# BrByte/brb_framework

Measured on AMD Instinct MI355X. Metric: GiB/s (device-resident) + Mrecords/s over 1500B buffers at 1/2/4/8 MI355X, higher is better.
Workload: dtype u32

## Files before the change

### brb_framework_amd/csrc/gpu/digest_line.h

```cpp
#pragma once

#include "dma_stage.h"
#include "test_options.h"

#ifndef BRB_LINE_PROBE
#define BRB_LINE_PROBE_DECL
#define BRB_LINE_PROBE(ev) ((void)0)
#endif

namespace brb_digest {

template <class Alg, bool OUT_ALIGNED, bool TAIL_HI>
BRB_DEV void line_finish(typename Alg::State &st, const uint32_t (&w0)[16], const uint32_t (&w1)[16],
                         const uint32_t (&tm)[16], const uint32_t (&tp)[16], uint32_t t, uint32_t rec_len,
                         uint8_t *out, uint64_t r, uint64_t n_rec)
{
    if (t == 0) {
        Alg::pad_only(st, rec_len);
        if (r < n_rec)
            Alg::template store<OUT_ALIGNED>(out, r, st);
        return;
    }
    uint32_t w[16];
#pragma unroll
    for (int i = 0; i < 16; i++)
        w[i] = ((TAIL_HI ? w1[i] : w0[i]) & tm[i]) | tp[i];
    Alg::finish(st, w, t, rec_len);
    if (r < n_rec)
        Alg::template store<OUT_ALIGNED>(out, r, st);
}

BRB_DEV void tail_masks(uint32_t t, uint32_t (&tm)[16], uint32_t (&tp)[16])
{
#pragma unroll
    for (uint32_t i = 0; i < 16; i++) {
        const uint32_t o = 4 * i;
        const uint32_t keep = t > o ? (t - o < 4 ? t - o : 4) : 0;
        tm[i] = uint32_t((uint64_t(1) << (8 * keep)) - 1);
        tp[i] = t >= o && t < o + 4 ? 0x80u << (8 * (t - o)) : 0u;
        asm volatile("" : "+v"(tm[i]), "+v"(tp[i]));
    }
}

inline bool line_tail_hi(uint32_t rec_len)
{
    return ((rec_len >> 6) & 1) != 0;
}

template <class Alg, int WAVES, bool OUT_ALIGNED, bool TAIL_HI>
__global__ __launch_bounds__(64 * WAVES, 2) void digest_line_kernel(const uint8_t *__restrict__ data,
                                                                             uint32_t rec_len, uint64_t n_rec,
                                                                             uint8_t *__restrict__ out)
{
    constexpr uint32_t SLOT = 8192;
    __shared__ __attribute__((aligned(16))) uint8_t ring[WAVES * 2 * SLOT];
    __shared__ uint32_t next_ticket;
    const uint32_t lane = threadIdx.x & 63;
    const uint32_t wv = __builtin_amdgcn_readfirstlane(threadIdx.x >> 6);
    [[maybe_unused]] const uint64_t wave0 = uint64_t(blockIdx.x) * WAVES + wv;
    const uint64_t n_groups = (n_rec + 63) / 64;
    if (threadIdx.x == 0)
        next_ticket = WAVES;
    __syncthreads();
    auto take = [&]() -> uint64_t {
        uint32_t tk = 0;
        if (lane == 0)
            tk = __hip_atomic_fetch_add(&next_ticket, 1u, __ATOMIC_RELAXED, __HIP_MEMORY_SCOPE_WORKGROUP);
        tk = __builtin_amdgcn_readfirstlane(tk);
        return uint64_t(blockIdx.x) + uint64_t(tk) * gridDim.x;
    };
    uint64_t g = uint64_t(blockIdx.x) + uint64_t(wv) * gridDim.x;
    if (g >= n_groups)
        return;
    const uint32_t my_off = wv * 2 * SLOT;
    const uint32_t lds0 = uint32_t(reinterpret_cast<uintptr_t>(ring)) + my_off;
    const uint32_t nfull = rec_len >> 6, t = rec_len & 63;
    const uint32_t nblk = nfull + (t ? 1 : 0);
    const uint32_t K = (nblk + 1) >> 1;
    const uint32_t P = (K & 1) ^ 1;
    const uint64_t dbase = reinterpret_cast<uint64_t>(data);
    const uint64_t end_line = (dbase + n_rec * rec_len + 127) & ~uint64_t(127);
    const uint64_t gbytes = uint64_t(rec_len) * 64;
    const uint32_t o0 = uint32_t(dbase) & 127;
    auto swz = [](uint32_t row) { return (row >> 1) & 7; };

    uint32_t vq[8];
    {
        const uint32_t l3 = lane >> 3;
        const uint32_t base = o0 + l3 * rec_len;
        const uint32_t g0 = 16u * ((lane & 7) ^ (l3 >> 1));
#pragma unroll
        for (int q = 0; q < 8; q++) {
            const uint32_t x = base + 8u * q * rec_len;
            vq[q] = ((x & ~127u) | (q & 1 ? g0 ^ 64u : g0)) + (4096u - 1024u * (q & 3));
        }
    }
    brb_dma::v4i rs, rsn;
    auto desc = [&](uint64_t g, brb_dma::v4i &rs) {
        const uint64_t gbase = ((dbase + g * gbytes) & ~uint64_t(127)) - 4096;
        const uint64_t gleft = end_line - gbase;
        rs.x = __builtin_amdgcn_readfirstlane(int(uint32_t(gbase)));
        rs.y = __builtin_amdgcn_readfirstlane(int(uint32_t(gbase >> 32) & 0xFFFF));
        rs.z = __builtin_amdgcn_readfirstlane(int(gleft > 0x7FFFFFFFull ? 0x7FFFFFFFu : uint32_t(gleft)));
        rs.w = 0x00020000;
    };
    uint32_t so = 0, son = 0;
    auto issue = [&](const brb_dma::v4i &rs, uint32_t &so, uint32_t slot, bool keep_l2 = false) {
#ifdef BRB_LINE_NO_DMA
        return;
#endif
        const uint32_t m = lds0 + slot * SLOT;
        uint32_t keep;
#define BRB_LINE_DMA8(POL)                                                                      \
    asm volatile("s_mov_b32 %0, m0\n\t"                                                          \
                 "s_mov_b32 m0, %10\n\t"                                                         \
                 "s_nop 0\n\t"                                                                   \
                 "buffer_load_dwordx4 %1, %9, %12 offen " POL "lds\n\t"                         \
                 "buffer_load_dwordx4 %2, %9, %12 offen offset:1024 " POL "lds\n\t"             \
                 "buffer_load_dwordx4 %3, %9, %12 offen offset:2048 " POL "lds\n\t"             \
                 "buffer_load_dwordx4 %4, %9, %12 offen offset:3072 " POL "lds\n\t"             \
                 "s_mov_b32 m0, %11\n\t"                                                         \
                 "s_nop 0\n\t"                                                                   \
                 "buffer_load_dwordx4 %5, %9, %12 offen " POL "lds\n\t"                         \
                 "buffer_load_dwordx4 %6, %9, %12 offen offset:1024 " POL "lds\n\t"             \
                 "buffer_load_dwordx4 %7, %9, %12 offen offset:2048 " POL "lds\n\t"             \
                 "buffer_load_dwordx4 %8, %9, %12 offen offset:3072 " POL "lds\n\t"             \
                 "s_mov_b32 m0, %0"                                                               \
                 : "=&s"(keep)                                                                    \
                 : "v"(vq[0]), "v"(vq[1]), "v"(vq[2]), "v"(vq[3]), "v"(vq[4]), "v"(vq[5]), "v"(vq[6]), \
                   "v"(vq[7]), "s"(rs), "s"(m), "s"(m + 4096u), "s"(so)                           \
                 : "memory")
        if (!keep_l2)
            BRB_LINE_DMA8("nt ");
        else
            BRB_LINE_DMA8("");
#undef BRB_LINE_DMA8
        so += 128;
    };

    uint32_t ae[32], ao[32];

    uint32_t w0[16], w1[16];
    auto read_window = [&](const uint32_t (&ad)[32]) {
#pragma unroll
        for (int i = 0; i < 16; i++) {
            w0[i] = *reinterpret_cast<const uint32_t *>(ring + ad[i]);
            w1[i] = *reinterpret_cast<const uint32_t *>(ring + ad[16 + i]);
        }
        __builtin_amdgcn_s_waitcnt(0xC07F);
    };

    BRB_LINE_PROBE_DECL
    BRB_LINE_PROBE(0);
    desc(g, rs);
    issue(rs, so, P, true);
    issue(rs, so, P ^ 1, true);
    __builtin_amdgcn_sched_barrier(0);
    uint64_t gn = take();
    {
        const uint32_t sh4 = (o0 + lane * rec_len) & 127;
        const uint32_t fr = (my_off + lane * 128) | (swz(lane) << 4);
#pragma unroll
        for (uint32_t i = 0; i < 32; i++) {
            const uint32_t q4 = sh4 + 4 * i;
            ae[i] = ((q4 & 124u) ^ fr) | ((q4 & 128u) << 6);
            ao[i] = ae[i] ^ SLOT;
            asm volatile("" : "+v"(ae[i]), "+v"(ao[i]));
        }
    }
    uint32_t tm[16], tp[16];
    tail_masks(t, tm, tp);
    auto full_step = [&](typename Alg::State &st, const uint32_t (&ad)[32], uint32_t refill_slot) {
        BRB_LINE_PROBE(1);
        brb_dma::wait_vmcnt<0>();
        read_window(ad);
        BRB_LINE_PROBE(2);
        issue(rs, so, refill_slot);
        __builtin_amdgcn_sched_barrier(0);
        Alg::compress(st, w0);
        Alg::compress(st, w1);
        __builtin_amdgcn_sched_barrier(0);
    };
    for (;;) {
        typename Alg::State st = Alg::iv();
        uint32_t k = 1;
        if (P) {
            full_step(st, ao, 1);
            k = 2;
        }
        for (; k + 2 <= K; k += 2) {
            full_step(st, ae, 0);
            full_step(st, ao, 1);
        }
        {
            BRB_LINE_PROBE(1);
            brb_dma::wait_vmcnt<0>();
            read_window(ae);
            BRB_LINE_PROBE(2);
            if (gn < n_groups) {
                desc(gn, rsn);
                son = 0;
                issue(rsn, son, P, true);
                issue(rsn, son, P ^ 1, true);
            }
            if (2 * K - 2 < nfull)
                Alg::compress(st, w0);
            if (2 * K - 1 < nfull)
                Alg::compress(st, w1);
        }
        line_finish<Alg, OUT_ALIGNED, TAIL_HI>(st, w0, w1, tm, tp, t, rec_len, out, g * 64 + lane, n_rec);
        g = gn;
        if (g >= n_groups)
            break;
        gn = take();
        rs = rsn;
        so = son;
    }
    BRB_LINE_PROBE(3);
}

inline bool line_supported(const uint8_t *data, uint32_t rec_len)
{
    return rec_len > 64 && rec_len <= (1u << 20) && (rec_len & 3) == 0 && (reinterpret_cast<uintptr_t>(data) & 3) == 0;
}

inline unsigned device_cu_count()
{
    static const unsigned n = [] {
        int dev = 0, c = 0;
        if (hipGetDevice(&dev) != hipSuccess || hipDeviceGetAttribute(&c, hipDeviceAttributeMultiprocessorCount, dev) != hipSuccess || c <= 0)
            c = 256;
        return unsigned(c);
    }();
    return n;
}

template <class Alg>
hipError_t launch_fixed_line(const uint8_t *data, uint32_t rec_len, uint64_t n_rec, uint8_t *out, bool out_al,
                             hipStream_t s)
{
    constexpr int W = 8;
    const uint64_t groups = (n_rec + 63) / 64;
    const unsigned g = unsigned(groups < device_cu_count() ? groups : device_cu_count());
    const bool hi = line_tail_hi(rec_len);
    if (out_al && hi)
        digest_line_kernel<Alg, W, true, true><<<g, 64 * W, 0, s>>>(data, rec_len, n_rec, out);
    else if (out_al)
        digest_line_kernel<Alg, W, true, false><<<g, 64 * W, 0, s>>>(data, rec_len, n_rec, out);
    else if (hi)
        digest_line_kernel<Alg, W, false, true><<<g, 64 * W, 0, s>>>(data, rec_len, n_rec, out);
    else
        digest_line_kernel<Alg, W, false, false><<<g, 64 * W, 0, s>>>(data, rec_len, n_rec, out);
    return hipGetLastError();
}

}
```

### brb_framework_amd/csrc/gpu/md5_device.h

```cpp
#pragma once

#include "brb_gpu_common.h"

#define BRB_MD5_F1(x, y, z) ((z) ^ ((x) & ((y) ^ (z))))
#define BRB_MD5_F2(x, y, z) ((y) ^ ((z) & ((x) ^ (y))))
#define BRB_MD5_F3(x, y, z) __builtin_amdgcn_bitop3_b32((x), (y), (z), 0x96)
#define BRB_MD5_F4(x, y, z) ((y) ^ ((x) | ~(z)))
#define BRB_MD5_STEP(F, a, b, c, d, m, k, s) (a) = (b) + rotl<s>((a) + F((b), (c), (d)) + ((m) + (k)))

struct Md5State {
    uint32_t a, b, c, d;
};

BRB_DEV Md5State md5_iv()
{
    return Md5State{0x67452301u, 0xefcdab89u, 0x98badcfeu, 0x10325476u};
}

#define BRB_MD5_STEP3X(a, b, c, d, m, k, s)                                               \
    do {                                                                                 \
        const uint32_t x_ = (a) + (m) + (k), cd_ = (c) ^ (d);                            \
        uint32_t f_;                                                                     \
        asm("v_xad_u32 %0, %1, %2, %3" : "=v"(f_) : "v"(b), "v"(cd_), "v"(x_));          \
        (a) = (b) + rotl<s>(f_);                                                         \
    } while (0)

template <bool XAD = true>
BRB_DEV void md5_compress(Md5State &st, const uint32_t (&m)[16])
{
    uint32_t a = st.a, b = st.b, c = st.c, d = st.d;

    BRB_MD5_STEP(BRB_MD5_F1, a, b, c, d, m[0], 0xd76aa478u, 7);
    BRB_MD5_STEP(BRB_MD5_F1, d, a, b, c, m[1], 0xe8c7b756u, 12);
    BRB_MD5_STEP(BRB_MD5_F1, c, d, a, b, m[2], 0x242070dbu, 17);
    BRB_MD5_STEP(BRB_MD5_F1, b, c, d, a, m[3], 0xc1bdceeeu, 22);
    BRB_MD5_STEP(BRB_MD5_F1, a, b, c, d, m[4], 0xf57c0fafu, 7);
    BRB_MD5_STEP(BRB_MD5_F1, d, a, b, c, m[5], 0x4787c62au, 12);
    BRB_MD5_STEP(BRB_MD5_F1, c, d, a, b, m[6], 0xa8304613u, 17);
    BRB_MD5_STEP(BRB_MD5_F1, b, c, d, a, m[7], 0xfd469501u, 22);
    BRB_MD5_STEP(BRB_MD5_F1, a, b, c, d, m[8], 0x698098d8u, 7);
    BRB_MD5_STEP(BRB_MD5_F1, d, a, b, c, m[9], 0x8b44f7afu, 12);
    BRB_MD5_STEP(BRB_MD5_F1, c, d, a, b, m[10], 0xffff5bb1u, 17);
    BRB_MD5_STEP(BRB_MD5_F1, b, c, d, a, m[11], 0x895cd7beu, 22);
    BRB_MD5_STEP(BRB_MD5_F1, a, b, c, d, m[12], 0x6b901122u, 7);
    BRB_MD5_STEP(BRB_MD5_F1, d, a, b, c, m[13], 0xfd987193u, 12);
    BRB_MD5_STEP(BRB_MD5_F1, c, d, a, b, m[14], 0xa679438eu, 17);
    BRB_MD5_STEP(BRB_MD5_F1, b, c, d, a, m[15], 0x49b40821u, 22);

    BRB_MD5_STEP(BRB_MD5_F2, a, b, c, d, m[1], 0xf61e2562u, 5);
    BRB_MD5_STEP(BRB_MD5_F2, d, a, b, c, m[6], 0xc040b340u, 9);
    BRB_MD5_STEP(BRB_MD5_F2, c, d, a, b, m[11], 0x265e5a51u, 14);
    BRB_MD5_STEP(BRB_MD5_F2, b, c, d, a, m[0], 0xe9b6c7aau, 20);
    BRB_MD5_STEP(BRB_MD5_F2, a, b, c, d, m[5], 0xd62f105du, 5);
    BRB_MD5_STEP(BRB_MD5_F2, d, a, b, c, m[10], 0x02441453u, 9);
    BRB_MD5_STEP(BRB_MD5_F2, c, d, a, b, m[15], 0xd8a1e681u, 14);
    BRB_MD5_STEP(BRB_MD5_F2, b, c, d, a, m[4], 0xe7d3fbc8u, 20);
    BRB_MD5_STEP(BRB_MD5_F2, a, b, c, d, m[9], 0x21e1cde6u, 5);
    BRB_MD5_STEP(BRB_MD5_F2, d, a, b, c, m[14], 0xc33707d6u, 9);
    BRB_MD5_STEP(BRB_MD5_F2, c, d, a, b, m[3], 0xf4d50d87u, 14);
    BRB_MD5_STEP(BRB_MD5_F2, b, c, d, a, m[8], 0x455a14edu, 20);
    BRB_MD5_STEP(BRB_MD5_F2, a, b, c, d, m[13], 0xa9e3e905u, 5);
    BRB_MD5_STEP(BRB_MD5_F2, d, a, b, c, m[2], 0xfcefa3f8u, 9);
    BRB_MD5_STEP(BRB_MD5_F2, c, d, a, b, m[7], 0x676f02d9u, 14);
    BRB_MD5_STEP(BRB_MD5_F2, b, c, d, a, m[12], 0x8d2a4c8au, 20);

    if constexpr (XAD) BRB_MD5_STEP3X(a, b, c, d, m[5], 0xfffa3942u, 4); else BRB_MD5_STEP(BRB_MD5_F3, a, b, c, d, m[5], 0xfffa3942u, 4);
    if constexpr (XAD) BRB_MD5_STEP3X(d, a, b, c, m[8], 0x8771f681u, 11); else BRB_MD5_STEP(BRB_MD5_F3, d, a, b, c, m[8], 0x8771f681u, 11);
    if constexpr (XAD) BRB_MD5_STEP3X(c, d, a, b, m[11], 0x6d9d6122u, 16); else BRB_MD5_STEP(BRB_MD5_F3, c, d, a, b, m[11], 0x6d9d6122u, 16);
    if constexpr (XAD) BRB_MD5_STEP3X(b, c, d, a, m[14], 0xfde5380cu, 23); else BRB_MD5_STEP(BRB_MD5_F3, b, c, d, a, m[14], 0xfde5380cu, 23);
    if constexpr (XAD) BRB_MD5_STEP3X(a, b, c, d, m[1], 0xa4beea44u, 4); else BRB_MD5_STEP(BRB_MD5_F3, a, b, c, d, m[1], 0xa4beea44u, 4);
    if constexpr (XAD) BRB_MD5_STEP3X(d, a, b, c, m[4], 0x4bdecfa9u, 11); else BRB_MD5_STEP(BRB_MD5_F3, d, a, b, c, m[4], 0x4bdecfa9u, 11);
    if constexpr (XAD) BRB_MD5_STEP3X(c, d, a, b, m[7], 0xf6bb4b60u, 16); else BRB_MD5_STEP(BRB_MD5_F3, c, d, a, b, m[7], 0xf6bb4b60u, 16);
    if constexpr (XAD) BRB_MD5_STEP3X(b, c, d, a, m[10], 0xbebfbc70u, 23); else BRB_MD5_STEP(BRB_MD5_F3, b, c, d, a, m[10], 0xbebfbc70u, 23);
    if constexpr (XAD) BRB_MD5_STEP3X(a, b, c, d, m[13], 0x289b7ec6u, 4); else BRB_MD5_STEP(BRB_MD5_F3, a, b, c, d, m[13], 0x289b7ec6u, 4);
    if constexpr (XAD) BRB_MD5_STEP3X(d, a, b, c, m[0], 0xeaa127fau, 11); else BRB_MD5_STEP(BRB_MD5_F3, d, a, b, c, m[0], 0xeaa127fau, 11);
    if constexpr (XAD) BRB_MD5_STEP3X(c, d, a, b, m[3], 0xd4ef3085u, 16); else BRB_MD5_STEP(BRB_MD5_F3, c, d, a, b, m[3], 0xd4ef3085u, 16);
    if constexpr (XAD) BRB_MD5_STEP3X(b, c, d, a, m[6], 0x04881d05u, 23); else BRB_MD5_STEP(BRB_MD5_F3, b, c, d, a, m[6], 0x04881d05u, 23);
    if constexpr (XAD) BRB_MD5_STEP3X(a, b, c, d, m[9], 0xd9d4d039u, 4); else BRB_MD5_STEP(BRB_MD5_F3, a, b, c, d, m[9], 0xd9d4d039u, 4);
    if constexpr (XAD) BRB_MD5_STEP3X(d, a, b, c, m[12], 0xe6db99e5u, 11); else BRB_MD5_STEP(BRB_MD5_F3, d, a, b, c, m[12], 0xe6db99e5u, 11);
    if constexpr (XAD) BRB_MD5_STEP3X(c, d, a, b, m[15], 0x1fa27cf8u, 16); else BRB_MD5_STEP(BRB_MD5_F3, c, d, a, b, m[15], 0x1fa27cf8u, 16);
    if constexpr (XAD) BRB_MD5_STEP3X(b, c, d, a, m[2], 0xc4ac5665u, 23); else BRB_MD5_STEP(BRB_MD5_F3, b, c, d, a, m[2], 0xc4ac5665u, 23);

    BRB_MD5_STEP(BRB_MD5_F4, a, b, c, d, m[0], 0xf4292244u, 6);
    BRB_MD5_STEP(BRB_MD5_F4, d, a, b, c, m[7], 0x432aff97u, 10);
    BRB_MD5_STEP(BRB_MD5_F4, c, d, a, b, m[14], 0xab9423a7u, 15);
    BRB_MD5_STEP(BRB_MD5_F4, b, c, d, a, m[5], 0xfc93a039u, 21);
    BRB_MD5_STEP(BRB_MD5_F4, a, b, c, d, m[12], 0x655b59c3u, 6);
    BRB_MD5_STEP(BRB_MD5_F4, d, a, b, c, m[3], 0x8f0ccc92u, 10);
    BRB_MD5_STEP(BRB_MD5_F4, c, d, a, b, m[10], 0xffeff47du, 15);
    BRB_MD5_STEP(BRB_MD5_F4, b, c, d, a, m[1], 0x85845dd1u, 21);
    BRB_MD5_STEP(BRB_MD5_F4, a, b, c, d, m[8], 0x6fa87e4fu, 6);
    BRB_MD5_STEP(BRB_MD5_F4, d, a, b, c, m[15], 0xfe2ce6e0u, 10);
    BRB_MD5_STEP(BRB_MD5_F4, c, d, a, b, m[6], 0xa3014314u, 15);
    BRB_MD5_STEP(BRB_MD5_F4, b, c, d, a, m[13], 0x4e0811a1u, 21);
    BRB_MD5_STEP(BRB_MD5_F4, a, b, c, d, m[4], 0xf7537e82u, 6);
    BRB_MD5_STEP(BRB_MD5_F4, d, a, b, c, m[11], 0xbd3af235u, 10);
    BRB_MD5_STEP(BRB_MD5_F4, c, d, a, b, m[2], 0x2ad7d2bbu, 15);
    BRB_MD5_STEP(BRB_MD5_F4, b, c, d, a, m[9], 0xeb86d391u, 21);

    st.a += a;
    st.b += b;
    st.c += c;
    st.d += d;
}

BRB_DEV void md5_finish(Md5State &st, uint32_t (&w)[16], uint32_t t, uint64_t total_len)
{
    if (t >= 56) {
        md5_compress(st, w);
#pragma unroll
        for (int i = 0; i < 14; i++)
            w[i] = 0;
    }
    w[14] = uint32_t(total_len << 3);
    w[15] = uint32_t(total_len >> 29);
    md5_compress(st, w);
}

BRB_DEV void md5_pad_only(Md5State &st, uint64_t total_len)
{
    uint32_t w[16] = {0x80u};
    w[14] = uint32_t(total_len << 3);
    w[15] = uint32_t(total_len >> 29);
    md5_compress<false>(st, w);
}
```

Baseline: 4571.

## Group records into alignment classes for vector LDS window reads; pair MD5 round-3 steps

Records are split into p alignment classes, chosen from rec_len mod 16, and each block is assigned one class. Within a class, every lane's record starts at the same 16-byte phase, so the LDS window can be read with 8-9 uint4 loads instead of 32 scalar dword loads. The phase is dispatched through compile-time specialisations, and the DMA source and window addresses are recomputed to keep the swizzle. MD5 round 3 also pairs consecutive steps so they share the b^c term. The change adds code size, more register use from the 36-word buffer, and a more complex grid mapping that could unbalance work across CUs.

```diff
diff --git a/brb_framework_amd/csrc/gpu/digest_line.h b/brb_framework_amd/csrc/gpu/digest_line.h
--- a/brb_framework_amd/csrc/gpu/digest_line.h
+++ b/brb_framework_amd/csrc/gpu/digest_line.h
@@ -1,6 +1,9 @@
 #pragma once
 
+#include <type_traits>
+
 #include "dma_stage.h"
+#include "line_layout.h"
 #include "test_options.h"
 
 #ifndef BRB_LINE_PROBE
@@ -52,13 +55,16 @@
                                                                              uint32_t rec_len, uint64_t n_rec,
                                                                              uint8_t *__restrict__ out)
 {
-    constexpr uint32_t SLOT = 8192;
+    constexpr uint32_t SLOT = brb_line_layout::kSlot;
     __shared__ __attribute__((aligned(16))) uint8_t ring[WAVES * 2 * SLOT];
     __shared__ uint32_t next_ticket;
     const uint32_t lane = threadIdx.x & 63;
     const uint32_t wv = __builtin_amdgcn_readfirstlane(threadIdx.x >> 6);
     [[maybe_unused]] const uint64_t wave0 = uint64_t(blockIdx.x) * WAVES + wv;
-    const uint64_t n_groups = (n_rec + 63) / 64;
+    const uint32_t p = brb_line_layout::period(rec_len);
+    const brb_line_layout::BlockMap bm = brb_line_layout::block_map(blockIdx.x, gridDim.x, p);
+    const uint64_t n_teams = brb_line_layout::team_count(n_rec, p);
+    const uint64_t tbytes = uint64_t(rec_len) * 64 * p;
     if (threadIdx.x == 0)
         next_ticket = WAVES;
     __syncthreads();
@@ -67,10 +73,11 @@
         if (lane == 0)
             tk = __hip_atomic_fetch_add(&next_ticket, 1u, __ATOMIC_RELAXED, __HIP_MEMORY_SCOPE_WORKGROUP);
         tk = __builtin_amdgcn_readfirstlane(tk);
-        return uint64_t(blockIdx.x) + uint64_t(tk) * gridDim.x;
-    };
-    uint64_t g = uint64_t(blockIdx.x) + uint64_t(wv) * gridDim.x;
-    if (g >= n_groups)
+        return uint64_t(bm.u) + uint64_t(tk) * bm.streams;
+    };
+    auto has_group = [&](uint64_t team) { return team < n_teams && team * 64 * p + bm.c < n_rec; };
+    uint64_t g = uint64_t(bm.u) + uint64_t(wv) * bm.streams;
+    if (!has_group(g))
         return;
     const uint32_t my_off = wv * 2 * SLOT;
     const uint32_t lds0 = uint32_t(reinterpret_cast<uintptr_t>(ring)) + my_off;
@@ -80,24 +87,18 @@
     const uint32_t P = (K & 1) ^ 1;
     const uint64_t dbase = reinterpret_cast<uint64_t>(data);
     const uint64_t end_line = (dbase + n_rec * rec_len + 127) & ~uint64_t(127);
-    const uint64_t gbytes = uint64_t(rec_len) * 64;
-    const uint32_t o0 = uint32_t(dbase) & 127;
-    auto swz = [](uint32_t row) { return (row >> 1) & 7; };
+    const uint64_t cbase = dbase + uint64_t(bm.c) * rec_len;
+    const uint32_t oc = brb_line_layout::class_off(uint32_t(dbase) & 127, bm.c, rec_len);
+    const uint32_t rstride = p * rec_len;
+    const uint32_t d = __builtin_amdgcn_readfirstlane(brb_line_layout::phase(oc));
 
     uint32_t vq[8];
-    {
-        const uint32_t l3 = lane >> 3;
-        const uint32_t base = o0 + l3 * rec_len;
-        const uint32_t g0 = 16u * ((lane & 7) ^ (l3 >> 1));
-#pragma unroll
-        for (int q = 0; q < 8; q++) {
-            const uint32_t x = base + 8u * q * rec_len;
-            vq[q] = ((x & ~127u) | (q & 1 ? g0 ^ 64u : g0)) + (4096u - 1024u * (q & 3));
-        }
-    }
+#pragma unroll
+    for (int q = 0; q < 8; q++)
+        vq[q] = brb_line_layout::dma_src(oc, rstride, q, lane) + (4096u - 1024u * (q & 3));
     brb_dma::v4i rs, rsn;
-    auto desc = [&](uint64_t g, brb_dma::v4i &rs) {
-        const uint64_t gbase = ((dbase + g * gbytes) & ~uint64_t(127)) - 4096;
+    auto desc = [&](uint64_t team, brb_dma::v4i &rs) {
+        const uint64_t gbase = ((cbase + team * tbytes) & ~uint64_t(127)) - 4096;
         const uint64_t gleft = end_line - gbase;
         rs.x = __builtin_amdgcn_readfirstlane(int(uint32_t(gbase)));
         rs.y = __builtin_amdgcn_readfirstlane(int(uint32_t(gbase >> 32) & 0xFFFF));
@@ -138,16 +139,29 @@
         so += 128;
     };
 
-    uint32_t ae[32], ao[32];
+    uint32_t ae[8], ao[8];
 
     uint32_t w0[16], w1[16];
-    auto read_window = [&](const uint32_t (&ad)[32]) {
-#pragma unroll
-        for (int i = 0; i < 16; i++) {
-            w0[i] = *reinterpret_cast<const uint32_t *>(ring + ad[i]);
-            w1[i] = *reinterpret_cast<const uint32_t *>(ring + ad[16 + i]);
+    auto read_window = [&](auto dtag, const uint32_t (&ad)[8], uint32_t ad8) {
+        constexpr int D = decltype(dtag)::value;
+        uint32_t buf[36];
+#pragma unroll
+        for (int j = 0; j < (D ? 9 : 8); j++) {
+            const uint4 v = *reinterpret_cast<const uint4 *>(ring + (j < 8 ? ad[j & 7] : ad8));
+            buf[4 * j] = v.x;
+            buf[4 * j + 1] = v.y;
+            buf[4 * j + 2] = v.z;
+            buf[4 * j + 3] = v.w;
         }
         __builtin_amdgcn_s_waitcnt(0xC07F);
+        if (D)
+            asm volatile("" : "+v"(buf[0]), "+v"(buf[1]), "+v"(buf[2]), "+v"(buf[3]), "+v"(buf[32]), "+v"(buf[33]),
+                         "+v"(buf[34]), "+v"(buf[35]));
+#pragma unroll
+        for (int i = 0; i < 16; i++) {
+            w0[i] = buf[D + i];
+            w1[i] = buf[D + 16 + i];
+        }
     };
 
     BRB_LINE_PROBE_DECL
@@ -157,64 +171,68 @@
     issue(rs, so, P ^ 1, true);
     __builtin_amdgcn_sched_barrier(0);
     uint64_t gn = take();
-    {
-        const uint32_t sh4 = (o0 + lane * rec_len) & 127;
-        const uint32_t fr = (my_off + lane * 128) | (swz(lane) << 4);
-#pragma unroll
-        for (uint32_t i = 0; i < 32; i++) {
-            const uint32_t q4 = sh4 + 4 * i;
-            ae[i] = ((q4 & 124u) ^ fr) | ((q4 & 128u) << 6);
-            ao[i] = ae[i] ^ SLOT;
-            asm volatile("" : "+v"(ae[i]), "+v"(ao[i]));
-        }
+#pragma unroll
+    for (uint32_t j = 0; j < 8; j++) {
+        ae[j] = my_off + brb_line_layout::win_addr(oc, rstride, lane, j);
+        ao[j] = ae[j] ^ SLOT;
+        asm volatile("" : "+v"(ae[j]), "+v"(ao[j]));
     }
     uint32_t tm[16], tp[16];
     tail_masks(t, tm, tp);
-    auto full_step = [&](typename Alg::State &st, const uint32_t (&ad)[32], uint32_t refill_slot) {
-        BRB_LINE_PROBE(1);
-        brb_dma::wait_vmcnt<0>();
-        read_window(ad);
-        BRB_LINE_PROBE(2);
-        issue(rs, so, refill_slot);
-        __builtin_amdgcn_sched_barrier(0);
-        Alg::compress(st, w0);
-        Alg::compress(st, w1);
-        __builtin_amdgcn_sched_barrier(0);
-    };
-    for (;;) {
-        typename Alg::State st = Alg::iv();
-        uint32_t k = 1;
-        if (P) {
-            full_step(st, ao, 1);
-            k = 2;
-        }
-        for (; k + 2 <= K; k += 2) {
-            full_step(st, ae, 0);
-            full_step(st, ao, 1);
-        }
-        {
+    auto run = [&](auto dtag) {
+        auto full_step = [&](typename Alg::State &st, const uint32_t (&ad)[8], uint32_t ad8, uint32_t refill_slot) {
             BRB_LINE_PROBE(1);
             brb_dma::wait_vmcnt<0>();
-            read_window(ae);
+            read_window(dtag, ad, ad8);
             BRB_LINE_PROBE(2);
-            if (gn < n_groups) {
-                desc(gn, rsn);
-                son = 0;
-                issue(rsn, son, P, true);
-                issue(rsn, son, P ^ 1, true);
+            issue(rs, so, refill_slot);
+            __builtin_amdgcn_sched_barrier(0);
+            Alg::compress(st, w0);
+            Alg::compress(st, w1);
+            __builtin_amdgcn_sched_barrier(0);
+        };
+        for (;;) {
+            typename Alg::State st = Alg::iv();
+            uint32_t k = 1;
+            if (P) {
+                full_step(st, ao, ae[0], 1);
+                k = 2;
             }
-            if (2 * K - 2 < nfull)
-                Alg::compress(st, w0);
-            if (2 * K - 1 < nfull)
-                Alg::compress(st, w1);
+            for (; k + 2 <= K; k += 2) {
+                full_step(st, ae, ao[0], 0);
+                full_step(st, ao, ae[0], 1);
+            }
+            {
+                BRB_LINE_PROBE(1);
+                brb_dma::wait_vmcnt<0>();
+                read_window(dtag, ae, ao[0]);
+                BRB_LINE_PROBE(2);
+                if (has_group(gn)) {
+                    desc(gn, rsn);
+                    son = 0;
+                    issue(rsn, son, P, true);
+                    issue(rsn, son, P ^ 1, true);
+                }
+                if (2 * K - 2 < nfull)
+                    Alg::compress(st, w0);
+                if (2 * K - 1 < nfull)
+                    Alg::compress(st, w1);
+            }
+            line_finish<Alg, OUT_ALIGNED, TAIL_HI>(st, w0, w1, tm, tp, t, rec_len, out,
+                                                   brb_line_layout::record_of(p, g, bm.c, lane), n_rec);
+            g = gn;
+            if (!has_group(g))
+                break;
+            gn = take();
+            rs = rsn;
+            so = son;
         }
-        line_finish<Alg, OUT_ALIGNED, TAIL_HI>(st, w0, w1, tm, tp, t, rec_len, out, g * 64 + lane, n_rec);
-        g = gn;
-        if (g >= n_groups)
-            break;
-        gn = take();
-        rs = rsn;
-        so = son;
+    };
+    switch (d) {
+    case 0: run(std::integral_constant<int, 0>{}); break;
+    case 1: run(std::integral_constant<int, 1>{}); break;
+    case 2: run(std::integral_constant<int, 2>{}); break;
+    default: run(std::integral_constant<int, 3>{}); break;
     }
     BRB_LINE_PROBE(3);
 }
@@ -240,8 +258,8 @@
                              hipStream_t s)
 {
     constexpr int W = 8;
-    const uint64_t groups = (n_rec + 63) / 64;
-    const unsigned g = unsigned(groups < device_cu_count() ? groups : device_cu_count());
+    const uint32_t p = brb_line_layout::period(rec_len);
+    const unsigned g = brb_line_layout::grid_for(brb_line_layout::team_count(n_rec, p), p, device_cu_count());
     const bool hi = line_tail_hi(rec_len);
     if (out_al && hi)
         digest_line_kernel<Alg, W, true, true><<<g, 64 * W, 0, s>>>(data, rec_len, n_rec, out);
diff --git a/brb_framework_amd/csrc/gpu/line_layout.h b/brb_framework_amd/csrc/gpu/line_layout.h
--- /dev/null
+++ b/brb_framework_amd/csrc/gpu/line_layout.h
@@ -0,0 +1,93 @@
+#pragma once
+
+#include <stdint.h>
+
+#if defined(__HIPCC__) || defined(__CUDACC__)
+#define BRB_LAYOUT_HD __host__ __device__ inline
+#else
+#define BRB_LAYOUT_HD inline
+#endif
+
+namespace brb_line_layout {
+
+constexpr uint32_t kLine = 128;
+constexpr uint32_t kSlot = 64 * kLine;
+
+BRB_LAYOUT_HD uint32_t period(uint32_t rec_len)
+{
+    return (rec_len & 15) == 0 ? 1u : (rec_len & 7) == 0 ? 2u : 4u;
+}
+
+BRB_LAYOUT_HD uint64_t team_count(uint64_t n_rec, uint32_t p)
+{
+    return (n_rec + 64 * p - 1) / (64 * uint64_t(p));
+}
+
+BRB_LAYOUT_HD uint64_t record_of(uint32_t p, uint64_t s, uint32_t c, uint32_t l)
+{
+    return 64 * uint64_t(p) * s + uint64_t(p) * l + c;
+}
+
+BRB_LAYOUT_HD uint32_t class_off(uint32_t o0, uint32_t c, uint32_t rec_len)
+{
+    return (o0 + c * (rec_len & 127)) & 127;
+}
+
+BRB_LAYOUT_HD uint32_t phase(uint32_t oc)
+{
+    return (oc & 15) >> 2;
+}
+
+BRB_LAYOUT_HD uint32_t row_x(uint32_t oc, uint32_t row, uint32_t rs)
+{
+    return oc + row * rs;
+}
+
+BRB_LAYOUT_HD uint32_t dma_dst(uint32_t q, uint32_t lane)
+{
+    return 1024 * q + 16 * lane;
+}
+
+BRB_LAYOUT_HD uint32_t dma_src(uint32_t oc, uint32_t rs, uint32_t q, uint32_t lane)
+{
+    const uint32_t row = 8 * q + (lane >> 3), pg = lane & 7;
+    const uint32_t x = row_x(oc, row, rs);
+    const uint32_t gr = (x & 127) >> 4;
+    return (x & ~127u) | (((pg - (row >> 1) + gr) & 7) << 4);
+}
+
+BRB_LAYOUT_HD uint32_t win_addr(uint32_t oc, uint32_t rs, uint32_t l, uint32_t j)
+{
+    const uint32_t gl = (row_x(oc, l, rs) & 127) >> 4;
+    return l * kLine + ((((l >> 1) + j) & 7) << 4) + (gl + j >= 8 ? kSlot : 0);
+}
+
+struct BlockMap {
+    uint32_t c, u, streams;
+};
+
+BRB_LAYOUT_HD BlockMap block_map(uint32_t b, uint32_t grid, uint32_t p)
+{
+    BlockMap m;
+    m.streams = grid / p;
+    if (grid % (8 * p) == 0) {
+        const uint32_t idx = b >> 3;
+        m.c = idx % p;
+        m.u = (idx / p) * 8 + (b & 7);
+    } else {
+        m.c = b % p;
+        m.u = b / p;
+    }
+    return m;
+}
+
+BRB_LAYOUT_HD uint32_t grid_for(uint64_t n_teams, uint32_t p, uint32_t cus)
+{
+    uint64_t cap = cus / p ? cus / p : 1;
+    if (cap >= 8)
+        cap &= ~uint64_t(7);
+    const uint64_t want = n_teams >= 8 ? (n_teams + 7) & ~uint64_t(7) : n_teams;
+    return uint32_t(want < cap ? want : cap) * p;
+}
+
+}
diff --git a/brb_framework_amd/csrc/gpu/md5_device.h b/brb_framework_amd/csrc/gpu/md5_device.h
--- a/brb_framework_amd/csrc/gpu/md5_device.h
+++ b/brb_framework_amd/csrc/gpu/md5_device.h
@@ -17,12 +17,15 @@
     return Md5State{0x67452301u, 0xefcdab89u, 0x98badcfeu, 0x10325476u};
 }
 
-#define BRB_MD5_STEP3X(a, b, c, d, m, k, s)                                               \
+#define BRB_MD5_STEP3P(a, b, c, d, m0, k0, s0, m1, k1, s1)                                \
     do {                                                                                 \
-        const uint32_t x_ = (a) + (m) + (k), cd_ = (c) ^ (d);                            \
+        const uint32_t x0_ = (a) + (m0) + (k0), bc_ = (b) ^ (c);                         \
         uint32_t f_;                                                                     \
-        asm("v_xad_u32 %0, %1, %2, %3" : "=v"(f_) : "v"(b), "v"(cd_), "v"(x_));          \
-        (a) = (b) + rotl<s>(f_);                                                         \
+        asm("v_xad_u32 %0, %1, %2, %3" : "=v"(f_) : "v"(bc_), "v"(d), "v"(x0_));         \
+        (a) = (b) + rotl<s0>(f_);                                                        \
+        const uint32_t x1_ = (d) + (m1) + (k1);                                          \
+        asm("v_xad_u32 %0, %1, %2, %3" : "=v"(f_) : "v"(a), "v"(bc_), "v"(x1_));         \
+        (d) = (a) + rotl<s1>(f_);                                                        \
     } while (0)
 
 template <bool XAD = true>
@@ -64,22 +67,33 @@
     BRB_MD5_STEP(BRB_MD5_F2, c, d, a, b, m[7], 0x676f02d9u, 14);
     BRB_MD5_STEP(BRB_MD5_F2, b, c, d, a, m[12], 0x8d2a4c8au, 20);
 
-    if constexpr (XAD) BRB_MD5_STEP3X(a, b, c, d, m[5], 0xfffa3942u, 4); else BRB_MD5_STEP(BRB_MD5_F3, a, b, c, d, m[5], 0xfffa3942u, 4);
-    if constexpr (XAD) BRB_MD5_STEP3X(d, a, b, c, m[8], 0x8771f681u, 11); else BRB_MD5_STEP(BRB_MD5_F3, d, a, b, c, m[8], 0x8771f681u, 11);
-    if constexpr (XAD) BRB_MD5_STEP3X(c, d, a, b, m[11], 0x6d9d6122u, 16); else BRB_MD5_STEP(BRB_MD5_F3, c, d, a, b, m[11], 0x6d9d6122u, 16);
-    if constexpr (XAD) BRB_MD5_STEP3X(b, c, d, a, m[14], 0xfde5380cu, 23); else BRB_MD5_STEP(BRB_MD5_F3, b, c, d, a, m[14], 0xfde5380cu, 23);
-    if constexpr (XAD) BRB_MD5_STEP3X(a, b, c, d, m[1], 0xa4beea44u, 4); else BRB_MD5_STEP(BRB_MD5_F3, a, b, c, d, m[1], 0xa4beea44u, 4);
-    if constexpr (XAD) BRB_MD5_STEP3X(d, a, b, c, m[4], 0x4bdecfa9u, 11); else BRB_MD5_STEP(BRB_MD5_F3, d, a, b, c, m[4], 0x4bdecfa9u, 11);
-    if constexpr (XAD) BRB_MD5_STEP3X(c, d, a, b, m[7], 0xf6bb4b60u, 16); else BRB_MD5_STEP(BRB_MD5_F3, c, d, a, b, m[7], 0xf6bb4b60u, 16);
-    if constexpr (XAD) BRB_MD5_STEP3X(b, c, d, a, m[10], 0xbebfbc70u, 23); else BRB_MD5_STEP(BRB_MD5_F3, b, c, d, a, m[10], 0xbebfbc70u, 23);
-    if constexpr (XAD) BRB_MD5_STEP3X(a, b, c, d, m[13], 0x289b7ec6u, 4); else BRB_MD5_STEP(BRB_MD5_F3, a, b, c, d, m[13], 0x289b7ec6u, 4);
-    if constexpr (XAD) BRB_MD5_STEP3X(d, a, b, c, m[0], 0xeaa127fau, 11); else BRB_MD5_STEP(BRB_MD5_F3, d, a, b, c, m[0], 0xeaa127fau, 11);
-    if constexpr (XAD) BRB_MD5_STEP3X(c, d, a, b, m[3], 0xd4ef3085u, 16); else BRB_MD5_STEP(BRB_MD5_F3, c, d, a, b, m[3], 0xd4ef3085u, 16);
-    if constexpr (XAD) BRB_MD5_STEP3X(b, c, d, a, m[6], 0x04881d05u, 23); else BRB_MD5_STEP(BRB_MD5_F3, b, c, d, a, m[6], 0x04881d05u, 23);
-    if constexpr (XAD) BRB_MD5_STEP3X(a, b, c, d, m[9], 0xd9d4d039u, 4); else BRB_MD5_STEP(BRB_MD5_F3, a, b, c, d, m[9], 0xd9d4d039u, 4);
-    if constexpr (XAD) BRB_MD5_STEP3X(d, a, b, c, m[12], 0xe6db99e5u, 11); else BRB_MD5_STEP(BRB_MD5_F3, d, a, b, c, m[12], 0xe6db99e5u, 11);
-    if constexpr (XAD) BRB_MD5_STEP3X(c, d, a, b, m[15], 0x1fa27cf8u, 16); else BRB_MD5_STEP(BRB_MD5_F3, c, d, a, b, m[15], 0x1fa27cf8u, 16);
-    if constexpr (XAD) BRB_MD5_STEP3X(b, c, d, a, m[2], 0xc4ac5665u, 23); else BRB_MD5_STEP(BRB_MD5_F3, b, c, d, a, m[2], 0xc4ac5665u, 23);
+    if constexpr (XAD) {
+        BRB_MD5_STEP3P(a, b, c, d, m[5], 0xfffa3942u, 4, m[8], 0x8771f681u, 11);
+        BRB_MD5_STEP3P(c, d, a, b, m[11], 0x6d9d6122u, 16, m[14], 0xfde5380cu, 23);
+        BRB_MD5_STEP3P(a, b, c, d, m[1], 0xa4beea44u, 4, m[4], 0x4bdecfa9u, 11);
+        BRB_MD5_STEP3P(c, d, a, b, m[7], 0xf6bb4b60u, 16, m[10], 0xbebfbc70u, 23);
+        BRB_MD5_STEP3P(a, b, c, d, m[13], 0x289b7ec6u, 4, m[0], 0xeaa127fau, 11);
+        BRB_MD5_STEP3P(c, d, a, b, m[3], 0xd4ef3085u, 16, m[6], 0x04881d05u, 23);
+        BRB_MD5_STEP3P(a, b, c, d, m[9], 0xd9d4d039u, 4, m[12], 0xe6db99e5u, 11);
+        BRB_MD5_STEP3P(c, d, a, b, m[15], 0x1fa27cf8u, 16, m[2], 0xc4ac5665u, 23);
+    } else {
+        BRB_MD5_STEP(BRB_MD5_F3, a, b, c, d, m[5], 0xfffa3942u, 4);
+        BRB_MD5_STEP(BRB_MD5_F3, d, a, b, c, m[8], 0x8771f681u, 11);
+        BRB_MD5_STEP(BRB_MD5_F3, c, d, a, b, m[11], 0x6d9d6122u, 16);
+        BRB_MD5_STEP(BRB_MD5_F3, b, c, d, a, m[14], 0xfde5380cu, 23);
+        BRB_MD5_STEP(BRB_MD5_F3, a, b, c, d, m[1], 0xa4beea44u, 4);
+        BRB_MD5_STEP(BRB_MD5_F3, d, a, b, c, m[4], 0x4bdecfa9u, 11);
+        BRB_MD5_STEP(BRB_MD5_F3, c, d, a, b, m[7], 0xf6bb4b60u, 16);
+        BRB_MD5_STEP(BRB_MD5_F3, b, c, d, a, m[10], 0xbebfbc70u, 23);
+        BRB_MD5_STEP(BRB_MD5_F3, a, b, c, d, m[13], 0x289b7ec6u, 4);
+        BRB_MD5_STEP(BRB_MD5_F3, d, a, b, c, m[0], 0xeaa127fau, 11);
+        BRB_MD5_STEP(BRB_MD5_F3, c, d, a, b, m[3], 0xd4ef3085u, 16);
+        BRB_MD5_STEP(BRB_MD5_F3, b, c, d, a, m[6], 0x04881d05u, 23);
+        BRB_MD5_STEP(BRB_MD5_F3, a, b, c, d, m[9], 0xd9d4d039u, 4);
+        BRB_MD5_STEP(BRB_MD5_F3, d, a, b, c, m[12], 0xe6db99e5u, 11);
+        BRB_MD5_STEP(BRB_MD5_F3, c, d, a, b, m[15], 0x1fa27cf8u, 16);
+        BRB_MD5_STEP(BRB_MD5_F3, b, c, d, a, m[2], 0xc4ac5665u, 23);
+    }
 
     BRB_MD5_STEP(BRB_MD5_F4, a, b, c, d, m[0], 0xf4292244u, 6);
     BRB_MD5_STEP(BRB_MD5_F4, d, a, b, c, m[7], 0x432aff97u, 10);
```

New measurement: 4613 (median of 6 runs). About the same (+0.9%).
